# phonism/genrec

Hardware: NVIDIA H100
Metric: hstu_train_sequences_per_sec (higher is better)
Workload: dtype bf16

## Files before the change

### genrec_b200/_lib.py

```python
from __future__ import annotations

import ctypes as C
import os
from typing import Optional

import torch

_HERE = os.path.dirname(os.path.abspath(__file__))
LIB_PATH = os.path.join(_HERE, "libgenrec_b200.so")

c_void_p, c_int, c_float, c_size_t = C.c_void_p, C.c_int, C.c_float, C.c_size_t
c_u64, c_i64, c_u32 = C.c_uint64, C.c_int64, C.c_uint32


class HstuDims(C.Structure):
    _fields_ = [("B", c_int), ("L", c_int), ("D", c_int), ("H", c_int), ("npos", c_int), ("ntime", c_int),
                ("dropout_p", c_float), ("seed", c_u64), ("seed_dev", c_void_p), ("layer_index", c_int)]


class HstuLayerParams(C.Structure):
    _fields_ = [(n, c_void_p) for n in ("proj_w", "proj_b", "pos_table", "time_table", "ln1_g", "ln1_b", "ffn1_w",
                                         "ffn1_b", "ffn2_w", "ffn2_b", "ln2_g", "ln2_b")]


# ... 5 lines not shown
class HstuLayerGrads(C.Structure):
    _fields_ = [(n, c_void_p) for n in ("proj_w", "proj_b", "pos_table", "time_table", "ln1_g", "ln1_b", "ffn1_w",
                                         "ffn1_b", "ffn2_w", "ffn2_b", "ln2_g", "ln2_b")]


class HstuSeq(C.Structure):
    _fields_ = [("bias_index", c_void_p), ("ld_index", c_int), ("has_time", c_int), ("pos_uniform", c_int), ("pos_bucket0", c_int)]


class HstuCache(C.Structure):
    _fields_ = [("B", c_int), ("capacity", c_int), ("num_layers", c_int), ("kv", c_void_p), ("timestamps", c_void_p),
                ("lengths", c_void_p), ("overflow", c_void_p)]


class HstuPool(C.Structure):
    _fields_ = [("max_users", c_int), ("num_layers", c_int), ("page_size", c_int), ("num_pages", c_int), ("max_items", c_int),
                ("kv", c_void_p), ("timestamps", c_void_p), ("page_table", c_void_p), ("lengths", c_void_p), ("overflow", c_void_p),
                ("free_stack", c_void_p), ("free_top", c_void_p), ("errors", c_void_p), ("row_of", c_void_p)]


class SasrecDims(C.Structure):
    _fields_ = [("B", c_int), ("L", c_int), ("D", c_int), ("H", c_int), ("dropout_p", c_float), ("seed", c_u64),
                ("seed_dev", c_void_p), ("layer_index", c_int)]


P = C.POINTER
SIGNATURES = {
    "grb_last_error": (C.c_char_p, []),
    "grb_version": (c_int, []),
    "grb_launch_count": (c_u64, []),
    "grb_check_device": (c_int, [c_int]),
    "grb_set_defer_weight_grads": (c_int, [c_int]),
    "grb_join_deferred": (c_int, [c_void_p]),
    "grb_hstu_layer_saved_bytes": (c_size_t, [P(HstuDims)]),
    "grb_hstu_layer_workspace_bytes": (c_size_t, [P(HstuDims)]),
    "grb_hstu_layer_forward": (c_int, [P(HstuDims), P(HstuLayerParams), P(HstuSeq), c_void_p, c_void_p, c_void_p, c_void_p]),
    "grb_hstu_layer_backward": (c_int, [P(HstuDims), P(HstuLayerParams), P(HstuSeq), c_void_p, c_void_p, c_void_p,
                                        P(HstuLayerGrads), c_void_p, c_void_p]),
    "grb_hstu_bias_index": (c_int, [c_void_p, c_void_p, c_void_p, c_void_p, c_int, c_int, c_int, c_int, c_void_p, c_int, c_void_p]),
    "grb_hstu_attention_scratch_bytes": (c_size_t, [P(HstuDims)]),
    "grb_hstu_attention_forward": (c_int, [P(HstuDims), c_void_p, c_void_p, P(HstuSeq), c_void_p, c_void_p, c_void_p]),
    "grb_hstu_attention_backward": (c_int, [P(HstuDims), c_void_p, c_void_p, P(HstuSeq), c_void_p, c_void_p, c_void_p, c_void_p,
                                            c_void_p, c_void_p, c_void_p, c_void_p]),
    "grb_hstu_cache_append": (c_int, [P(HstuCache), c_void_p, c_void_p, c_int, c_void_p, c_void_p, c_void_p]),
    "grb_hstu_layer_extend_workspace_bytes": (c_size_t, [P(HstuDims), c_int]),
    "grb_hstu_layer_extend": (c_int, [P(HstuDims), P(HstuLayerParams), P(HstuCache), c_int, c_void_p, c_void_p, c_int, c_void_p,
                                      c_void_p, c_void_p, c_void_p, c_void_p]),
    "grb_hstu_pool_append": (c_int, [P(HstuPool), c_void_p, c_int, c_void_p, c_void_p, c_int, c_void_p, c_void_p, c_void_p, c_void_p]),
    "grb_hstu_pool_release": (c_int, [P(HstuPool), c_void_p, c_int, c_void_p, c_int, c_void_p]),
    "grb_hstu_layer_extend_paged_workspace_bytes": (c_size_t, [P(HstuDims), P(HstuPool)]),
    "grb_hstu_layer_extend_paged": (c_int, [P(HstuDims), P(HstuLayerParams), P(HstuPool), c_int, c_void_p, c_void_p, c_void_p, c_int,
                                            c_void_p, c_void_p, c_void_p, c_void_p, c_void_p]),
    "grb_collate_jagged": (c_int, [c_void_p, c_void_p, c_void_p, c_void_p, c_int, c_int, c_void_p, c_void_p, c_void_p, c_void_p]),
    "grb_embed_forward": (c_int, [c_void_p, c_void_p, c_void_p, c_void_p, c_void_p, c_int, c_int, c_int, c_float, c_int,
                                  c_float, c_u64, c_void_p, c_void_p]),
    "grb_embed_backward": (c_int, [c_void_p, c_void_p, c_void_p, c_void_p, c_void_p, c_int, c_int, c_int, c_float, c_int, c_float,
                                   c_u64, c_void_p, c_void_p, c_void_p]),
    "grb_head_workspace_bytes": (c_size_t, [c_int, c_int, c_int]),
    "grb_head_splits": (c_int, [c_int, c_int, c_int, c_int]),
    "grb_head_loss_forward_backward": (c_int, [c_void_p, c_void_p, c_void_p, c_float, c_void_p, c_void_p, c_int, c_int, c_int,
                                               c_void_p, c_void_p, c_void_p, c_void_p, c_void_p, c_void_p, c_void_p]),
    "grb_head_sampled_workspace_bytes": (c_size_t, [c_int, c_int, c_int]),
    "grb_head_sampled_loss_forward_backward": (c_int, [c_void_p, c_void_p, c_void_p, c_float, c_void_p, c_void_p, c_void_p, c_void_p,
                                                       c_int, c_int, c_int, c_int, c_void_p, c_void_p, c_void_p, c_void_p, c_void_p,
                                                       c_void_p, c_void_p]),
    "grb_head_logits": (c_int, [c_void_p, c_void_p, c_void_p, c_float, c_void_p, c_int, c_int, c_int, c_void_p, c_void_p,
# ... 124 lines not shown
```

### genrec_b200/csrc/api.cu

```cuda
#include "../../include/genrec_b200.h"

#include <cstdarg>
#include <cstdio>
#include <cstring>
#include <initializer_list>
#include <mutex>
#include <type_traits>
#include <utility>

#include "attn_hstu.cuh"
#include "attn_hstu_extend.cuh"
#include "attn_sasrec.cuh"
#include "attn_t5.cuh"
#include "beam.cuh"
#include "common.cuh"
#include "dp_adam.cuh"
#include "exact_f32.cuh"
#include "head_candidates.cuh"
#include "head_rank.cuh"
#include "head_topk.cuh"
#include "lazy_adam.cuh"
#include "rowwise.cuh"
#include "rq_argmin.cuh"
#include "rq_sinkhorn.cuh"
// ... 102 lines not shown
    const int need = (T + ROW_THREADS / 32 - 1) / (ROW_THREADS / 32), cap = sm_count() * 3;
    return need < cap ? (need < 1 ? 1 : need) : cap;
}
dim3 colsum_grid(int T, int N) {
    const int cx = (N + 255) / 256, maxy = (T + 63) / 64;
    int cy = (4 * sm_count() + cx - 1) / cx;
    cy = cy > maxy ? maxy : cy;
    return dim3(cx, cy < 1 ? 1 : cy);
}
dim3 cast_colsum_grid(int T, int D) {
    const int cx = (D + 127) / 128, maxy = (T + 31) / 32;
    int cy = (8 * sm_count() + cx - 1) / cx;
    cy = cy > maxy ? maxy : cy;
    return dim3(cx, cy < 1 ? 1 : cy);
}
size_t attn_dw_part_floats(int B, int L, int H) { return (size_t)2 * H * B * ((L + ATT_BLK - 1) / ATT_BLK) * 64; }
struct DetOut {
    float* out;
    int len;
};
int det_finish(const float* part, int ngroups, int nmembers, int W, int gpo, int gstride, int estride, std::initializer_list<DetOut> outs,
               cudaStream_t st) {
    DetFinishArgs f;
    memset(&f, 0, sizeof(f));
    f.part = part; f.ngroups = ngroups; f.nmembers = nmembers; f.W = W; f.gpo = gpo; f.gstride = gstride; f.estride = estride;
    int k = 0;
    for (const DetOut& o : outs) { f.out[k] = o.out; f.len[k] = o.len; ++k; }
    const unsigned blocks = (unsigned)(((size_t)ngroups * W * 32 + 255) / 256);
    launch_k(det_finish_kernel, blocks, 256, 0, st, f);
    GRB_CUDA(cudaGetLastError());
    return 0;
}

cudaError_t gemm_bias_act(int act, const bf16* x, const bf16* w, const float* bias, bf16* z, bf16* a, int M, int N, int K, const Dropout& drop,
                          cudaStream_t st) {
    if (act == 0) return launch_tc_gemm<0>(x, w, M, N, K, K, K, TcEpiBiasAct<0>{bias, N, drop}, z, nullptr, N, sm_count(), st);
    if (act == 1) return launch_tc_gemm<0>(x, w, M, N, K, K, K, TcEpiBiasAct<1>{bias, N, drop}, z, a, N, sm_count(), st);
    return launch_tc_gemm<0>(x, w, M, N, K, K, K, TcEpiBiasAct<2>{bias, N, drop}, z, a, N, sm_count(), st);
}
cudaError_t gemm_bias_res(const bf16* x, const bf16* w, const float* bias, const float* res, const float* row_scale, float* y, int M, int N,
                          int K, const Dropout& drop, cudaStream_t st) {
    return launch_tc_gemm<0>(x, w, M, N, K, K, K, TcEpiBiasResidual{bias, res, row_scale, N, drop}, y, nullptr, N, sm_count(), st);
}
cudaError_t gemm_dact(int act, const bf16* dy, const bf16* w, const bf16* z, bf16* g, int M, int N, int K, const Dropout& drop, cudaStream_t st) {
    if (act == 1) return launch_tc_gemm<1>(dy, w, M, N, K, K, N, TcEpiDAct<1>{z, N, drop}, g, nullptr, N, sm_count(), st);
    return launch_tc_gemm<1>(dy, w, M, N, K, K, N, TcEpiDAct<2>{z, N, drop}, g, nullptr, N, sm_count(), st);
}
cudaError_t gemm_nn_f32(const bf16* A, const bf16* B, float* out, const float* res, float scale, int M, int N, int K, int lda, int ldb,
                        cudaStream_t st) {
    return launch_tc_gemm<1>(A, B, M, N, K, lda, ldb, TcEpiF32{res, N, scale}, out, nullptr, N, sm_count(), st);
}

struct LayerSaved {
    bf16 *xb, *zp, *P, *O, *xn, *z1, *hact;
    float *st1, *x1, *st2;
    size_t bytes;
};
LayerSaved carve_saved(void* base, size_t T, size_t D) {
    LayerSaved s;
    Carver c{static_cast<char*>(base)};
    s.xb = c.take<bf16>(T * D * 2);
    s.zp = c.take<bf16>(T * 4 * D * 2);
    s.P = c.take<bf16>(T * 4 * D * 2);
    s.O = c.take<bf16>(T * D * 2);
    s.st1 = c.take<float>(T * 2 * 4);
    s.x1 = c.take<float>(T * D * 4);
    s.xn = c.take<bf16>(T * D * 2);
    s.st2 = c.take<float>(T * 2 * 4);
    s.z1 = c.take<bf16>(T * 4 * D * 2);
    s.hact = c.take<bf16>(T * 4 * D * 2);
    s.bytes = c.off;
    return s;
}
struct LayerWork {
    bf16 *dyb, *dz1, *dO, *dzp;
    float *dxn, *dx1;
    float *part_tn, *part_colsum, *part_cast, *part_ln, *part_attn;
    size_t bytes;
};
void layer_tn_specs(TnSpec (&specs)[3], const bf16* dyb, const bf16* hact, const bf16* dz1, const bf16* xn, const bf16* dzp, const bf16* xb,
                    float* dw2, float* dw1, float* dwp, int T, int D) {
    specs[0] = {dyb, hact, dw2, D, 4 * D, T, D, 4 * D, 4 * D};
    specs[1] = {dz1, xn, dw1, 4 * D, D, T, 4 * D, D, D};
// ... 110 lines not shown
struct SideStream {
    cudaStream_t s = nullptr;
    cudaEvent_t fork = nullptr, join = nullptr;
    bool ok = false, pending = false;
    template <class F>
    int run(cudaStream_t st, F&& launch) {
        if (!ok) {
            GRB_CUDA(cudaStreamCreateWithFlags(&s, cudaStreamNonBlocking));
            GRB_CUDA(cudaEventCreateWithFlags(&fork, cudaEventDisableTiming));
            GRB_CUDA(cudaEventCreateWithFlags(&join, cudaEventDisableTiming));
            ok = true;
        }
        GRB_CUDA(cudaEventRecord(fork, st));
        GRB_CUDA(cudaStreamWaitEvent(s, fork, 0));
        GRB_TRY(launch(s));
        GRB_CUDA(cudaEventRecord(join, s));
        pending = true;
        return 0;
    }
    int join_into(cudaStream_t st) {
        if (pending) {
            GRB_CUDA(cudaStreamWaitEvent(st, join, 0));
            pending = false;
        }
        return 0;
    }
};
SideStream& attn_side_stream() {
    static thread_local SideStream ss[64];
    return ss[current_device() & 63];
}
std::mutex g_defer_mu;
bool g_defer_on = false;
SideStream& defer_stream() {
    static SideStream ds[64];
    return ds[current_device() & 63];
}
template <class F>
int defer_run(cudaStream_t st, F&& launch) {
    std::lock_guard<std::mutex> lock(g_defer_mu);
    return defer_stream().run(st, launch);
}
int join_pending(cudaStream_t st) {
    std::lock_guard<std::mutex> lock(g_defer_mu);
    return defer_stream().join_into(st);
}
template <class F>
int run_maybe_deferred(cudaStream_t st, F&& launch) {
    if (g_defer_on) return defer_run(st, launch);
    return launch(st);
}

template <int DH>
int launch_hstu_attn_bwd(const HstuAttnArgs& a, cudaStream_t st) {
    dim3 grid((a.L + ATT_BLK - 1) / ATT_BLK, a.H, a.B);
    size_t posb = align_up((size_t)(a.bias.npos * 64 + 1) * 4, 16);
    size_t smem_q = sizeof(AttSmem<DH>) + posb;
    GRB_TRY(set_smem(hstu_attn_bwd_dq_kernel<DH>, smem_q));
    SideStream& ss = attn_side_stream();
    GRB_TRY(ss.run(st, [&](cudaStream_t side) -> int {
        launch_k(hstu_attn_bwd_dq_kernel<DH>, grid, ATT_THREADS, smem_q, side, a);
        GRB_CUDA(cudaGetLastError());
        return 0;
    }));
    const bool has_time = a.bias.wtime != nullptr && a.bias.ntime > 0, pos_uni = a.bias.pos_uniform != 0;
    size_t smem_k = sizeof(AttSmemKV<DH>) + posb +
                    (size_t)4 * (att_time_bins(has_time, pos_uni, a.bias.ntime) + (pos_uni ? 0 : a.bias.npos + 1)) * 32 * sizeof(float);
    const int nmem = (int)(grid.x * grid.z), ngroups = has_time && a.dwtime ? 2 * a.H : a.H;
    GRB_REQUIRE((pos_uni || a.bias.npos <= 64) && a.bias.ntime <= 64, "attention backward: at most 64 position / time buckets");
    auto go = [&](auto kern) -> int {
        GRB_TRY(set_smem(kern, smem_k));
        launch_k(kern, grid, ATT_THREADS, smem_k, st, a, (int)posb);
        return 0;
    };
    if (has_time && pos_uni) GRB_TRY(go(hstu_attn_bwd_dkdv_kernel<DH, true, true>));
    else if (has_time) GRB_TRY(go(hstu_attn_bwd_dkdv_kernel<DH, true, false>));
    else if (pos_uni) GRB_TRY(go(hstu_attn_bwd_dkdv_kernel<DH, false, true>));
    else GRB_TRY(go(hstu_attn_bwd_dkdv_kernel<DH, false, false>));
// ... 175 lines not shown
extern "C" {

const char* grb_last_error(void) { return g_err; }
int grb_version(void) { return 100; }
uint64_t grb_launch_count(void) { return (uint64_t)launch_counter(); }

int grb_check_device(int ordinal) {
    cudaDeviceProp prop;
    cudaError_t e = cudaGetDeviceProperties(&prop, ordinal);
    if (e != cudaSuccess) return fail(GRB_ENODEV, "cudaGetDeviceProperties(%d): %s", ordinal, cudaGetErrorString(e));
    if (prop.major != 9 || prop.minor != 0) return fail(GRB_ENODEV, "device %d is sm_%d%d; this library is built for sm_90a only", ordinal, prop.major, prop.minor);
    return 0;
}

size_t grb_hstu_layer_saved_bytes(const grb_hstu_dims* d) {
    if (check_dims(d)) return 0;
    return carve_saved(nullptr, (size_t)d->B * d->L, d->D).bytes;
}
size_t grb_hstu_layer_workspace_bytes(const grb_hstu_dims* d) {
    if (check_dims(d)) return 0;
    return carve_work(nullptr, d).bytes;
}

int grb_hstu_layer_forward(const grb_hstu_dims* d, const grb_hstu_layer_params* p, const grb_hstu_seq* s, const float* x,
                           float* y, void* saved, void* stream) {
    GRB_TRY(check_dims(d));
    GRB_REQUIRE(x && y && saved, "null argument");
    GRB_TRY(check_layer_params(p));
    GRB_TRY(check_seq(d, s));
    GRB_REQUIRE(aligned16(x) && aligned16(y) && aligned16(saved), "buffers must be 16-byte aligned");
    cudaStream_t st = static_cast<cudaStream_t>(stream);
    const int T = d->B * d->L, D = d->D;
    LayerSaved sv = carve_saved(saved, T, D);

    GRB_TRY(block_steps_in(p, x, sv, T, D, st));
    GRB_TRY(join_pending(st));
    HstuAttnArgs a = make_attn_args(d, p->pos_table, p->time_table, s, sv.P, sv.O);
    GRB_TRY(with_head_dim(D / d->H, [&](auto DH) { return launch_hstu_attn_fwd<DH>(a, st); }));
    return block_steps_out(p, x, y, sv, T, D, make_dropout(d->dropout_p, d->seed, site_of(d->layer_index, SITE_GATE), d->seed_dev),
                           make_dropout(d->dropout_p, d->seed, site_of(d->layer_index, SITE_FFN_HID), d->seed_dev),
                           make_dropout(d->dropout_p, d->seed, site_of(d->layer_index, SITE_FFN_OUT), d->seed_dev), st);
}

int grb_hstu_layer_backward(const grb_hstu_dims* d, const grb_hstu_layer_params* p, const grb_hstu_seq* s, const float* dy,
                            const void* saved, float* dx, const grb_hstu_layer_grads* g, void* workspace, void* stream) {
    GRB_TRY(check_dims(d));
    GRB_REQUIRE(p && dy && saved && dx && g && workspace, "null argument");
    GRB_TRY(check_seq(d, s));
    GRB_REQUIRE(g->proj_w && g->proj_b && g->pos_table && g->ln1_g && g->ln1_b && g->ffn1_w && g->ffn1_b && g->ffn2_w && g->ffn2_b &&
                    g->ln2_g && g->ln2_b, "null gradient pointer");
    GRB_REQUIRE(aligned16(dy) && aligned16(dx) && aligned16(saved) && aligned16(workspace), "buffers must be 16-byte aligned");
    cudaStream_t st = static_cast<cudaStream_t>(stream);
    const int T = d->B * d->L, D = d->D;
    LayerSaved sv = carve_saved(const_cast<void*>(saved), T, D);
    LayerWork w = carve_work(workspace, d);
    const Dropout drop_out = make_dropout(d->dropout_p, d->seed, site_of(d->layer_index, SITE_FFN_OUT), d->seed_dev);
    const Dropout drop_hid = make_dropout(d->dropout_p, d->seed, site_of(d->layer_index, SITE_FFN_HID), d->seed_dev);
    const Dropout drop_gate = make_dropout(d->dropout_p, d->seed, site_of(d->layer_index, SITE_GATE), d->seed_dev);

    GRB_TRY(cast_colsum(dy, w.dyb, T, D, drop_out, g->ffn2_b, w.part_cast, st));
    GRB_CUDA(gemm_dact(1, w.dyb, (const bf16*)p->ffn2_w, sv.z1, w.dz1, T, 4 * D, D, drop_hid, st));
    auto colsum_4d = [&](const bf16* in, float* out) {
        return run_maybe_deferred(st, [&](cudaStream_t s_) -> int { return colsum(in, T, 4 * D, 4 * D, out, w.part_colsum, s_); });
    };
    GRB_TRY(colsum_4d(w.dz1, g->ffn1_b));
    GRB_CUDA(gemm_nn_f32(w.dz1, (const bf16*)p->ffn1_w, w.dxn, nullptr, 1.f, T, D, 4 * D, 4 * D, D, st));
    {
        LnGateBwdArgs a{dy, w.dxn, sv.x1, sv.st1, sv.st2, sv.O, D, sv.P, 4 * D, sv.zp, 4 * D, p->ln1_g, p->ln1_b, p->ln2_g,
                        w.dx1, w.dO, D, w.dzp, 4 * D, g->ln1_g, g->ln1_b, g->ln2_g, g->ln2_b, T, D, drop_gate, w.part_ln};
        GRB_TRY(with_row_dim(D, [&](auto DC) { launch_k(ln_gate_bwd_kernel<DC / 64>, row_grid(T), ROW_THREADS, 0, st, a); }));
        GRB_TRY(det_finish(w.part_ln, 4, row_grid(T), D, 1, 0, 1, {{a.dg1, D}, {a.db1, D}, {a.dg2, D}, {a.db2, D}}, st));
    }
    {
        HstuAttnArgs a = make_attn_args(d, p->pos_table, p->time_table, s, sv.P, sv.O);
        GRB_TRY(set_attn_bwd_args(a, d, s, w.dO, sv.zp, w.dzp, g->pos_table, g->time_table, w.part_attn));
        GRB_TRY(with_head_dim(D / d->H, [&](auto DH) { return launch_hstu_attn_bwd<DH>(a, st); }));
    }
    GRB_TRY(colsum_4d(w.dzp, g->proj_b));
    GRB_CUDA(gemm_nn_f32(w.dzp, (const bf16*)p->proj_w, dx, w.dx1, 1.f, T, D, 4 * D, 4 * D, D, st));
    TnSpec specs[3];
    layer_tn_specs(specs, w.dyb, sv.hact, w.dz1, sv.xn, w.dzp, sv.xb, g->ffn2_w, g->ffn1_w, g->proj_w, T, D);
    return run_maybe_deferred(st, [&](cudaStream_t s_) -> int {
        GRB_CUDA(launch_tc_tn_group(specs, 3, sm_count(), w.part_tn, s_));
        return 0;
    });
}

int grb_hstu_cache_append(const grb_hstu_cache* c, const int64_t* input_ids, const int64_t* timestamps, int n, int32_t* positions,
                          int32_t* last_row, void* stream) {
    GRB_REQUIRE(c && input_ids && positions && last_row, "null argument");
    GRB_REQUIRE(c->timestamps && c->lengths && c->overflow, "null cache pointer");
    GRB_REQUIRE(c->B > 0 && n > 0, "bad shape B=%d n=%d", c->B, n);
    GRB_REQUIRE(c->capacity >= 1 && c->capacity <= 16384, "cache capacity %d out of range [1, 16384]", c->capacity);
    launch_k(hstu_cache_append_kernel, (unsigned)((c->B + 3) / 4), 128, 0, static_cast<cudaStream_t>(stream),
             reinterpret_cast<const long long*>(input_ids), reinterpret_cast<const long long*>(timestamps), (const long long*)nullptr,
             (const int*)nullptr, c->B, n, c->capacity, KvPages{nullptr, 1, c->capacity}, reinterpret_cast<long long*>(c->timestamps),
             c->lengths, c->overflow, positions, last_row);
    GRB_CUDA(cudaGetLastError());
    return 0;
}

int grb_hstu_pool_append(const grb_hstu_pool* pool, const int64_t* users, int B, const int64_t* input_ids, const int64_t* timestamps,
                         int n, int32_t* positions, int32_t* last_row, int32_t* room, void* stream) {
    GRB_TRY(check_pool(pool));
    GRB_REQUIRE(users && input_ids && positions && last_row && room, "null argument");
    GRB_REQUIRE(pool->timestamps && pool->page_table && pool->lengths && pool->overflow && pool->free_stack && pool->free_top &&
                    pool->errors && pool->row_of, "null pool pointer");
    GRB_REQUIRE(B > 0 && n > 0, "bad shape B=%d n=%d", B, n);
    cudaStream_t st = static_cast<cudaStream_t>(stream);
    HstuPoolArgs a = pool_args(pool, users, B);
    a.ids = reinterpret_cast<const long long*>(input_ids); a.n = n;
    a.room = room;
    launch_k(hstu_pool_alloc_kernel, 1, POOL_THREADS, 0, st, a);
    GRB_CUDA(cudaGetLastError());
    launch_k(hstu_cache_append_kernel, (unsigned)((B + 3) / 4), 128, 0, st, reinterpret_cast<const long long*>(input_ids),
             reinterpret_cast<const long long*>(timestamps), reinterpret_cast<const long long*>(users), (const int*)room, B, n,
// ... 46 lines not shown
                                const int64_t* time_thr, const float* x, float* y, void* workspace, void* stream) {
    GRB_TRY(check_pool(pool));
    GRB_TRY(check_extend(d, pool->max_items));
    GRB_REQUIRE(p && users && positions && x && y && workspace && pool->kv && pool->timestamps && pool->page_table, "null argument");
    GRB_REQUIRE(layer >= 0 && layer < pool->num_layers, "layer %d out of range [0, %d)", layer, pool->num_layers);
    ExtendKv kv{static_cast<bf16*>(pool->kv) + (size_t)layer * pool->num_pages * pool->page_size * 2 * d->D,
                reinterpret_cast<const long long*>(pool->timestamps), reinterpret_cast<const long long*>(users),
                KvPages{pool->page_table, pool_pt_ld(pool), pool->page_size}, pool->max_items};
    return layer_extend(d, p, kv, positions, pos_bucket, pos_bucket0, time_thr, x, y, workspace, static_cast<cudaStream_t>(stream));
}

int grb_hstu_bias_index(const int64_t* timestamps, const uint8_t* pad, const int64_t* time_thr, const uint8_t* pos_bucket, int B, int L,
                        int npos, int ntime, uint16_t* out, int ld_index, void* stream) {
    GRB_REQUIRE(pad && time_thr && pos_bucket && out, "null argument");
    GRB_REQUIRE(B > 0 && L > 0 && B <= 65535 && L <= 65535, "bad shape B=%d L=%d", B, L);
    GRB_REQUIRE(ld_index >= L && ld_index % 8 == 0, "ld_index must be a multiple of 8 and >= L");
    GRB_REQUIRE(ntime >= 0 && ntime <= ATT_MAX_BUCKETS && npos >= 1 && npos <= ATT_MAX_BUCKETS, "bucket counts out of range");
    dim3 grid((ld_index + 255) / 256, (L + 7) / 8, B);
    auto go = [&](cudaStream_t s_) -> int {
        launch_k(hstu_bias_index_kernel, grid, 256, 0, s_, reinterpret_cast<const long long*>(timestamps), pad,
                 reinterpret_cast<const long long*>(time_thr), pos_bucket, L, ld_index, npos, ntime, out);
        GRB_CUDA(cudaGetLastError());
        return 0;
    };
    return run_maybe_deferred(static_cast<cudaStream_t>(stream), go);
}

int grb_set_defer_weight_grads(int on) {
    std::lock_guard<std::mutex> lock(g_defer_mu);
    g_defer_on = on != 0;
    return 0;
}
int grb_join_deferred(void* stream) { return join_pending(static_cast<cudaStream_t>(stream)); }

size_t grb_hstu_attention_scratch_bytes(const grb_hstu_dims* d) {
    if (check_dims(d)) return 0;
    return align_up(attn_dw_part_floats(d->B, d->L, d->H) * sizeof(float));
}

int grb_hstu_attention_forward(const grb_hstu_dims* d, const float* pos_table, const float* time_table, const grb_hstu_seq* s,
                               const void* P_bf16, void* O_bf16, void* stream) {
    GRB_TRY(check_dims(d));
    GRB_REQUIRE(pos_table && P_bf16 && O_bf16, "null argument");
    GRB_TRY(check_seq(d, s));
    GRB_REQUIRE(aligned16(P_bf16) && aligned16(O_bf16), "buffers must be 16-byte aligned");
    HstuAttnArgs a = make_attn_args(d, pos_table, time_table, s, (const bf16*)P_bf16, (bf16*)O_bf16);
    return with_head_dim(d->D / d->H, [&](auto DH) { return launch_hstu_attn_fwd<DH>(a, static_cast<cudaStream_t>(stream)); });
}
int grb_hstu_attention_backward(const grb_hstu_dims* d, const float* pos_table, const float* time_table, const grb_hstu_seq* s,
                                const void* P_bf16, const void* zp_bf16, const void* dO_bf16, void* dzp_bf16, float* dpos_table,
                                float* dtime_table, void* scratch, void* stream) {
    GRB_TRY(check_dims(d));
    GRB_REQUIRE(pos_table && P_bf16 && dO_bf16 && dzp_bf16 && dpos_table && scratch, "null argument");
    GRB_TRY(check_seq(d, s));
    GRB_REQUIRE(aligned16(P_bf16) && aligned16(dO_bf16) && aligned16(dzp_bf16) && aligned16(scratch) && (zp_bf16 == nullptr || aligned16(zp_bf16)),
                "buffers must be 16-byte aligned");
    HstuAttnArgs a = make_attn_args(d, pos_table, time_table, s, (const bf16*)P_bf16, nullptr);
    GRB_TRY(set_attn_bwd_args(a, d, s, (const bf16*)dO_bf16, (const bf16*)zp_bf16, (bf16*)dzp_bf16, dpos_table, dtime_table,
                              static_cast<float*>(scratch)));
    return with_head_dim(d->D / d->H, [&](auto DH) { return launch_hstu_attn_bwd<DH>(a, static_cast<cudaStream_t>(stream)); });
}

int grb_collate_jagged(const int64_t* items, const int64_t* stamps, const int64_t* offsets, const int64_t* targets, int B, int L,
                       int64_t* out_input_ids, int64_t* out_targets, int64_t* out_timestamps, void* stream) {
    GRB_REQUIRE(items && offsets && targets && out_input_ids && out_targets, "null argument");
    GRB_REQUIRE(B > 0 && L > 0, "bad shape B=%d L=%d", B, L);
    const size_t n = (size_t)B * L;
    launch_k(collate_jagged_kernel, (unsigned)((n + 255) / 256), 256, 0, static_cast<cudaStream_t>(stream), reinterpret_cast<const long long*>(items),
             reinterpret_cast<const long long*>(stamps), reinterpret_cast<const long long*>(offsets), reinterpret_cast<const long long*>(targets), B, L,
             reinterpret_cast<long long*>(out_input_ids), reinterpret_cast<long long*>(out_targets), reinterpret_cast<long long*>(out_timestamps));
    GRB_CUDA(cudaGetLastError());
    return 0;
}

int grb_embed_forward(const int64_t* ids, const float* table, const float* pos_table, float* x, uint8_t* pad, int B, int L, int D,
                      float scale, int mask_pad_rows, float dropout_p, uint64_t seed, const uint64_t* seed_dev, void* stream) {
    GRB_REQUIRE(ids && table && x, "null argument");
    GRB_REQUIRE(B > 0 && L > 0 && D > 0 && D % 4 == 0, "bad shape");
    EmbedArgs a{reinterpret_cast<const long long*>(ids), table, pos_table, x, pad, B * L, L, D, scale, mask_pad_rows,
                make_dropout(dropout_p, seed, SITE_EMBED, seed_dev)};
    launch_k(embed_fwd_kernel, row_grid(B * L), ROW_THREADS, 0, static_cast<cudaStream_t>(stream), a);
    GRB_CUDA(cudaGetLastError());
    return 0;
}
int grb_embed_backward(const int64_t* ids, const int64_t* order, const float* dx, float* dtable, float* dpos_table, int B, int L, int D,
                       float scale, int mask_pad_rows, float dropout_p, uint64_t seed, const uint64_t* seed_dev, float* scratch, void* stream) {
    GRB_REQUIRE(ids && order && dx && dtable && scratch, "null argument");
    GRB_REQUIRE(D <= 128 * EMB_MAX_CH, "embedding backward supports D <= %d", 128 * EMB_MAX_CH);
    GRB_REQUIRE(D % 4 == 0 && aligned16(dx) && aligned16(dtable) && aligned16(scratch) && (dpos_table == nullptr || aligned16(dpos_table)),
                "embedding backward needs D %% 4 == 0 and 16-byte aligned buffers");
    EmbedBwdArgs a{reinterpret_cast<const long long*>(ids), dx, dtable, dpos_table, B * L, L, D, scale, mask_pad_rows,
                   make_dropout(dropout_p, seed, SITE_EMBED, seed_dev), reinterpret_cast<const long long*>(order)};
    const EmbedPieceArgs pa{a, scratch};
    launch_k(embed_bwd_piece_kernel, row_grid((B * L + 31) / 32), ROW_THREADS, 0, static_cast<cudaStream_t>(stream), pa);
    GRB_CUDA(cudaGetLastError());
    launch_k(embed_bwd_run_kernel, row_grid(B * L), ROW_THREADS, 0, static_cast<cudaStream_t>(stream), pa);
    GRB_CUDA(cudaGetLastError());
    if (dpos_table) {
        launch_k(embed_bwd_pos_kernel, L < 8 * sm_count() ? L : 8 * sm_count(), ROW_THREADS, 0, static_cast<cudaStream_t>(stream), a);
        GRB_CUDA(cudaGetLastError());
    }
    return 0;
}

namespace {
struct HeadCommon {
    bf16* xf; float* stf; float* dxf; float* scal;
    float* row_loss;
    float* shift;
    float* part_ln;
};
void carve_head_common(Carver& c, HeadCommon& h, size_t T, size_t D) {
    h.xf = c.take<bf16>(T * D * 2);
    h.stf = c.take<float>(T * 2 * 4);
    h.dxf = c.take<float>(T * D * 4);
    h.scal = c.take<float>(64);
    h.row_loss = c.take<float>(T * 4);
    h.shift = c.take<float>(T * 4);
    h.part_ln = c.take<float>((size_t)2 * row_bwd_grid((int)T) * D * 4);
}
struct HeadWork : HeadCommon {
    bf16* logits;
    float* logits32;
    float* part_tn;
    int *ce_rsched, *ce_tsched;
    float *ce_rcarry, *ce_tcarry;
// ... 32 lines not shown

size_t grb_head_workspace_bytes(int T, int D, int C) { return carve_head(nullptr, T, D, C).bytes; }
int grb_head_splits(int T, int D, int C, int table) {
    const HeadWork h = carve_head(nullptr, T, D, C);
    return table ? h.tseg : h.rseg;
}

int grb_head_loss_forward_backward(const float* x, const float* ln_g, const float* ln_b, float ln_eps, const void* table_bf16,
                                   const int64_t* targets, int T, int D, int C, float* loss, float* dx, float* dtable, float* dln_g,
                                   float* dln_b, void* workspace, void* stream) {
    GRB_REQUIRE(x && ln_g && ln_b && table_bf16 && targets && loss && workspace, "null argument");
    GRB_REQUIRE(T > 0 && C > 1 && (D == 64 || D == 128 || D == 256), "bad shape T=%d D=%d C=%d", T, D, C);
    const bool want_grad = dx != nullptr;
    GRB_REQUIRE(!want_grad || (dtable && dln_g && dln_b), "null gradient pointer");
    cudaStream_t st = static_cast<cudaStream_t>(stream);
    HeadWork h = carve_head(workspace, T, D, C);
    const bool count_aside = g_defer_on;
    auto count = [&](cudaStream_t s_) -> int {
        launch_k(ce_count_kernel, 1, 1024, 0, s_, reinterpret_cast<const long long*>(targets), T, h.scal, loss);
        GRB_CUDA(cudaGetLastError());
        return 0;
    };
    if (count_aside) GRB_TRY(defer_run(st, count));
    GRB_TRY(head_ln_forward(x, ln_g, ln_b, ln_eps, h.xf, h.stf, T, D, st));
    if (count_aside) GRB_TRY(join_pending(st));
    else GRB_TRY(count(st));
    if (head_fused(D)) {
        CeArgs ca{reinterpret_cast<const long long*>(targets), h.scal, T, C, want_grad ? h.dxf : nullptr, h.shift, h.row_loss, dtable,
                  h.rseg, h.tseg, h.ce_rsched, h.ce_tsched, h.ce_rcarry, h.ce_tcarry};
        GRB_CUDA(with_ce_dim(D, [&](auto DC) { return launch_tc_ce<DC>(h.xf, (const bf16*)table_bf16, ca, sm_count(), st); }));
        launch_k(ce_loss_sum_kernel, 1, 1024, 0, st, (const float*)h.row_loss, T, loss);
        GRB_CUDA(cudaGetLastError());
        if (!want_grad) return 0;
        GRB_TRY(run_maybe_deferred(st, [&](cudaStream_t s_) -> int {
            GRB_CUDA(with_ce_dim(D, [&](auto DC) { return launch_ce_table<DC>(h.xf, (const bf16*)table_bf16, ca, sm_count(), s_); }));
            return 0;
        }));
    } else {
        GRB_CUDA((launch_tc_gemm<0>(h.xf, (const bf16*)table_bf16, T, C, D, D, D, TcEpiF32{nullptr, h.ldl, 1.f}, h.logits32, nullptr, h.ldl,
                                    sm_count(), st)));
        if (h.ldl / 8 <= 256 * 8)
            launch_k(ce_fwd_bwd_vec_kernel<8>, T, 256, 0, st, h.logits, h.ldl, C, reinterpret_cast<const long long*>(targets), h.scal, h.row_loss, want_grad ? 1 : 0,
                     (const float*)h.logits32);
        else
            launch_k(ce_fwd_bwd_kernel, T, 256, 0, st, h.logits, h.ldl, C, reinterpret_cast<const long long*>(targets), h.scal, h.row_loss, want_grad ? 1 : 0,
                     (const float*)h.logits32);
        GRB_CUDA(cudaGetLastError());
        launch_k(ce_loss_sum_kernel, 1, 1024, 0, st, (const float*)h.row_loss, T, loss);
        GRB_CUDA(cudaGetLastError());
        if (!want_grad) return 0;
        GRB_CUDA(gemm_nn_f32(h.logits, (const bf16*)table_bf16, h.dxf, nullptr, 1.f, T, D, C, h.ldl, D, st));
        TnSpec spec{h.logits, h.xf, dtable, C, D, T, h.ldl, D, D};
        GRB_TRY(run_maybe_deferred(st, [&](cudaStream_t s_) -> int {
            GRB_CUDA(launch_tc_tn_group(&spec, 1, sm_count(), h.part_tn, s_));
            return 0;
        }));
    }
    return head_ln_backward(h, x, ln_g, dx, dln_g, dln_b, T, D, st);
}

namespace {
struct SampledWork : HeadCommon {
    bf16* Es; float* bias; int* sid;
    float *ztgt, *gtgt;
    float* part; int ks;
    int Npad;
    size_t bytes;
};
SampledWork carve_sampled(void* base, size_t T, size_t D, size_t N) {
    SampledWork h;
    Carver c{static_cast<char*>(base)};
    h.Npad = (int)((N + 63) / 64 * 64);
    h.ks = sce_table_splits((int)T, h.Npad, sm_count());
    carve_head_common(c, h, T, D);
    h.Es = c.take<bf16>((size_t)h.Npad * D * 2);
    h.bias = c.take<float>((size_t)h.Npad * 4);
    h.sid = c.take<int>((size_t)h.Npad * 4);
    h.ztgt = c.take<float>(T * 4);
    h.gtgt = c.take<float>(T * 4);
    h.part = c.take<float>((size_t)h.ks * h.Npad * D * 4);
    h.bytes = c.off;
    return h;
}
int check_sampled_shape(int T, int D, int N) {
    GRB_REQUIRE(T >= 1, "sampled head: T=%d must be >= 1", T);
    GRB_REQUIRE(D == 64 || D == 128, "sampled head: D=%d is not supported (D must be 64 or 128; D = 256 is served by the full head only)", D);
    GRB_REQUIRE(N >= 1 && N <= SCE_MAX_N, "sampled head: N=%d negatives, must be 1 .. %d", N, SCE_MAX_N);
    return 0;
}
// ... 348 lines not shown
    float *part_colsum, *part_tn;
    size_t bytes;
};
TnSpec linear_dw_spec(const void* dy_bf16, const void* x_bf16, float* dw, int T, int N, int K) {
    return TnSpec{(const bf16*)dy_bf16, (const bf16*)x_bf16, dw, N, K, T, N, K, K};
}
LinearBwdWork carve_linear_bwd(void* base, int T, int N, int K) {
    LinearBwdWork w;
    Carver c{static_cast<char*>(base)};
    const dim3 cg = colsum_grid(T, N);
    w.part_colsum = c.take<float>((size_t)cg.x * cg.y * 256 * 4);
    const TnSpec spec = linear_dw_spec(nullptr, nullptr, nullptr, T, N, K);
    w.part_tn = c.take<float>(tn_part_floats(&spec, 1, sm_count()) * 4);
    w.bytes = c.off;
    return w;
}
}

size_t grb_linear_backward_workspace_bytes(int T, int N, int K) {
    if (T <= 0 || N <= 0 || K <= 0) return 0;
    return carve_linear_bwd(nullptr, T, N, K).bytes;
}
int grb_linear_backward(const void* dy_bf16, const void* w_bf16, const void* x_bf16, int T, int N, int K, float* dx_f32,
                        const float* dx_residual, float* dw, float* db, void* workspace, void* stream) {
    GRB_REQUIRE(dy_bf16 && w_bf16, "null argument");
    GRB_REQUIRE(T > 0 && N % 8 == 0 && K % 8 == 0, "N and K must be multiples of 8");
    GRB_REQUIRE(workspace || (!dw && !db), "workspace is null");
    cudaStream_t st = static_cast<cudaStream_t>(stream);
    const LinearBwdWork w = carve_linear_bwd(workspace, T, N, K);
    if (db) GRB_TRY(colsum((const bf16*)dy_bf16, T, N, N, db, w.part_colsum, st));
    if (dw) {
        GRB_REQUIRE(x_bf16, "x is null");
        const TnSpec spec = linear_dw_spec(dy_bf16, x_bf16, dw, T, N, K);
        GRB_CUDA(launch_tc_tn_group(&spec, 1, sm_count(), w.part_tn, st));
    }
    if (dx_f32) {
        GRB_CUDA(gemm_nn_f32((const bf16*)dy_bf16, (const bf16*)w_bf16, dx_f32, dx_residual, 1.f, T, K, N, N, K, st));
    }
    return 0;
}

int grb_linear_dact_backward(const void* dy_bf16, const void* w_bf16, const void* z_bf16, int T, int N, int K, int act, float dropout_p,
                             uint64_t seed, const uint64_t* seed_dev, uint32_t site, void* g_bf16, void* stream) {
    GRB_REQUIRE(dy_bf16 && w_bf16 && z_bf16 && g_bf16, "null argument");
    GRB_REQUIRE(T > 0 && N % 8 == 0 && K % 8 == 0 && (act == 1 || act == 2), "bad argument");
    GRB_CUDA(gemm_dact(act, (const bf16*)dy_bf16, (const bf16*)w_bf16, (const bf16*)z_bf16, (bf16*)g_bf16, T, K, N,
                       make_dropout(dropout_p, seed, site, seed_dev), static_cast<cudaStream_t>(stream)));
    return 0;
}
int grb_cast_rows_f32_to_bf16(const float* in, void* out_bf16, int T, int D, const float* row_scale, float dropout_p, uint64_t seed,
                              const uint64_t* seed_dev, uint32_t site, void* stream) {
    GRB_REQUIRE(in && out_bf16 && T > 0 && D > 0 && D % 4 == 0, "bad argument");
    return cast_bf16(in, (bf16*)out_bf16, (size_t)T * D, D, make_dropout(dropout_p, seed, site, seed_dev), row_scale,
                     static_cast<cudaStream_t>(stream));
}

int grb_layernorm_forward(const float* x, const float* g, const float* b, float eps, int T, int D, void* y_bf16, float* y_f32,
                          float* stats, void* stream) {
    GRB_REQUIRE(x && g && b && (y_bf16 || y_f32), "null argument");
    LnFwdArgs a{x, g, b, (bf16*)y_bf16, y_f32, stats, T, D, eps};
    cudaStream_t st = static_cast<cudaStream_t>(stream);
    return with_row_dim(D, [&](auto DC) { launch_k(ln_fwd_kernel<DC / 64>, row_grid(T), ROW_THREADS, 0, st, a); });
}
size_t grb_layernorm_backward_workspace_bytes(int T, int D) {
    if (T <= 0 || D <= 0) return 0;
    return (size_t)2 * row_bwd_grid(T) * D * 4;
}
// ... 489 lines not shown
```

### genrec_b200/csrc/tc_tn_group.cuh

```cuda
#pragma once
#include "tc_gemm.cuh"

namespace grb {

constexpr int TN_MAX_PROBLEMS = 4;

struct TnProblem {
    int M, N, K;
    int num_m, num_n, splits, kb_total, kb_per_split;
    int work_begin;
    int part_begin;
    float* out;
    int ldo;
};
struct TnGroupParams {
    CUtensorMap tmA[TN_MAX_PROBLEMS];
    CUtensorMap tmB[TN_MAX_PROBLEMS];
    TnProblem p[TN_MAX_PROBLEMS];
    int nprob;
    int total_work;
    float* part;
};


// ... 149 lines not shown
    memset(&P, 0, sizeof(P));
    P.nprob = n;
    double total = 0;
    for (int i = 0; i < n; ++i) total += (double)specs[i].M * specs[i].N * specs[i].K;
    int work = 0, parts = 0;
    for (int i = 0; i < n; ++i) {
        const TnSpec& s = specs[i];
        TnProblem& q = P.p[i];
        q.M = s.M; q.N = s.N; q.K = s.K; q.out = s.out; q.ldo = s.ldo;
        q.num_m = (s.M + TC_BM - 1) / TC_BM;
        q.num_n = (s.N + TC_BN - 1) / TC_BN;
        q.kb_total = (s.K + TC_BK - 1) / TC_BK;
        const int tiles = q.num_m * q.num_n;
        int want_items = (int)(2.0 * num_sms * ((double)s.M * s.N * s.K / total) + 0.5);
        int splits = (want_items + tiles - 1) / tiles;
        if (splits < 1) splits = 1;
        int max_splits = q.kb_total / 4 > 0 ? q.kb_total / 4 : 1;
        if (splits > max_splits) splits = max_splits;
        q.kb_per_split = (q.kb_total + splits - 1) / splits;
        q.splits = (q.kb_total + q.kb_per_split - 1) / q.kb_per_split;
        q.work_begin = work;
        q.part_begin = q.splits > 1 ? parts : -1;
        work += tiles * q.splits;
        if (q.splits > 1) parts += tiles * q.splits;
    }
    P.total_work = work;
    return (size_t)parts * (TC_BM * TC_BN);
}
inline size_t tn_part_floats(const TnSpec* specs, int n, int num_sms) {
    TnGroupParams P;
    return n < 1 || n > TN_MAX_PROBLEMS ? 0 : tn_plan(P, specs, n, num_sms);
}

inline cudaError_t launch_tc_tn_group(const TnSpec* specs, int n, int num_sms, float* part, cudaStream_t st) {
    if (n < 1 || n > TN_MAX_PROBLEMS) return cudaErrorInvalidValue;
    TnGroupParams P;
    const size_t need = tn_plan(P, specs, n, num_sms);
    if (need > 0 && part == nullptr) return cudaErrorInvalidValue;
    P.part = part;
    for (int i = 0; i < n; ++i) {
        const TnSpec& s = specs[i];
        if (!make_tmap_bf16(&P.tmA[i], s.A, s.K, s.M, s.lda, 64, TC_BK) || !make_tmap_bf16(&P.tmB[i], s.B, s.K, s.N, s.ldb, 64, TC_BK))
            return cudaErrorInvalidValue;
    }
    const int work = P.total_work;
    cudaError_t e = set_max_smem(tc_tn_group_kernel, TN_SMEM_BYTES);
    if (e != cudaSuccess) return e;
    int grid = work < num_sms ? work : num_sms;
    launch_k(tc_tn_group_kernel, grid, TC_THREADS, TN_SMEM_BYTES, st, P);
    e = cudaGetLastError();
    if (e != cudaSuccess) return e;
    int tiles = 0;
    for (int i = 0; i < n; ++i)
        if (P.p[i].splits > 1) tiles += P.p[i].num_m * P.p[i].num_n;
    if (tiles == 0) return cudaSuccess;
    launch_k(tn_finish_kernel, tiles * TN_FINISH_SLABS, 256, 0, st, P);
    return cudaGetLastError();
}

}
```

### include/genrec_b200.h

```cpp
#ifndef GENREC_B200_H
#define GENREC_B200_H

#include <stddef.h>
#include <stdint.h>

#ifdef __cplusplus
extern "C" {
#endif

#define GRB_OK 0
#define GRB_EINVAL (-1)
#define GRB_ECUDA (-2)
#define GRB_ENODEV (-3)

const char* grb_last_error(void);
int grb_version(void);
uint64_t grb_launch_count(void);
int grb_check_device(int ordinal);

typedef struct {
    int B, L, D, H;
    int npos, ntime;
    float dropout_p;
    uint64_t seed;
// ... 11 lines not shown
    const void* ffn1_w;
    const float* ffn1_b;
    const void* ffn2_w;
    const float* ffn2_b;
    const float* ln2_g;
    const float* ln2_b;
} grb_hstu_layer_params;

typedef struct {
    float* proj_w; float* proj_b; float* pos_table; float* time_table;
    float* ln1_g; float* ln1_b; float* ffn1_w; float* ffn1_b; float* ffn2_w; float* ffn2_b; float* ln2_g; float* ln2_b;
} grb_hstu_layer_grads;

typedef struct {
    const uint16_t* bias_index;
    int ld_index;
    int has_time;
    int pos_uniform;
    int pos_bucket0;
} grb_hstu_seq;

size_t grb_hstu_attention_scratch_bytes(const grb_hstu_dims* d);
int grb_hstu_attention_forward(const grb_hstu_dims* d, const float* pos_table, const float* time_table, const grb_hstu_seq* s,
                               const void* P_bf16, void* O_bf16, void* stream);
int grb_hstu_attention_backward(const grb_hstu_dims* d, const float* pos_table, const float* time_table, const grb_hstu_seq* s,
                                const void* P_bf16, const void* zp_bf16, const void* dO_bf16, void* dzp_bf16, float* dpos_table,
                                float* dtime_table, void* scratch, void* stream);

int grb_hstu_bias_index(const int64_t* timestamps, const uint8_t* pad, const int64_t* time_thr, const uint8_t* pos_bucket, int B,
                        int L, int npos, int ntime, uint16_t* out, int ld_index, void* stream);

int grb_set_defer_weight_grads(int on);
int grb_join_deferred(void* stream);

size_t grb_hstu_layer_saved_bytes(const grb_hstu_dims* d);
size_t grb_hstu_layer_workspace_bytes(const grb_hstu_dims* d);
int grb_hstu_layer_forward(const grb_hstu_dims* d, const grb_hstu_layer_params* p, const grb_hstu_seq* s,
                           const float* x, float* y, void* saved, void* stream);
int grb_hstu_layer_backward(const grb_hstu_dims* d, const grb_hstu_layer_params* p, const grb_hstu_seq* s,
                            const float* dy, const void* saved, float* dx, const grb_hstu_layer_grads* g,
                            void* workspace, void* stream);

typedef struct {
    int B, capacity, num_layers;
    void* kv;
    int64_t* timestamps;
    int32_t* lengths;
    uint8_t* overflow;
} grb_hstu_cache;
int grb_hstu_cache_append(const grb_hstu_cache* c, const int64_t* input_ids, const int64_t* timestamps, int n, int32_t* positions,
                          int32_t* last_row, void* stream);
size_t grb_hstu_layer_extend_workspace_bytes(const grb_hstu_dims* d, int capacity);
int grb_hstu_layer_extend(const grb_hstu_dims* d, const grb_hstu_layer_params* p, const grb_hstu_cache* c, int layer,
                          const int32_t* positions, const uint8_t* pos_bucket, int pos_bucket0, const int64_t* time_thr,
                          const float* x, float* y, void* workspace, void* stream);

typedef struct {
    int max_users, num_layers;
    int page_size;
    int num_pages;
    int max_items;
    void* kv;
    int64_t* timestamps;
    int32_t* page_table;
    int32_t* lengths;
    uint8_t* overflow;
// ... 149 lines not shown
```

Before: 40590.

## Partition SMs between main stream and deferred side-stream weight-grad kernels

Adds an SM budget for deferred side-stream work (the CE table gradient and TN weight-grad groups). The budget is sized from a cost model comparing table-pass time with the remaining block-chain time, and the main-stream GEMMs now launch on the SMs left over. An event makes embedding backward wait for the table gradient. The aim is real overlap between the deferred table gradient and the backward chain instead of both competing for every SM. The risk is that the main GEMMs run on fewer SMs and that the hard-coded cost constants are miscalibrated for H100.

```diff
diff --git a/genrec_b200/_lib.py b/genrec_b200/_lib.py
--- a/genrec_b200/_lib.py
+++ b/genrec_b200/_lib.py
@@ -61,6 +61,7 @@
     "grb_check_device": (c_int, [c_int]),
     "grb_set_defer_weight_grads": (c_int, [c_int]),
     "grb_join_deferred": (c_int, [c_void_p]),
+    "grb_set_side_sm_budget": (c_int, [c_int]),
     "grb_hstu_layer_saved_bytes": (c_size_t, [P(HstuDims)]),
     "grb_hstu_layer_workspace_bytes": (c_size_t, [P(HstuDims)]),
     "grb_hstu_layer_forward": (c_int, [P(HstuDims), P(HstuLayerParams), P(HstuSeq), c_void_p, c_void_p, c_void_p, c_void_p]),
diff --git a/genrec_b200/csrc/api.cu b/genrec_b200/csrc/api.cu
--- a/genrec_b200/csrc/api.cu
+++ b/genrec_b200/csrc/api.cu
@@ -158,23 +158,25 @@
     return 0;
 }
 
+int main_sms();
+
 cudaError_t gemm_bias_act(int act, const bf16* x, const bf16* w, const float* bias, bf16* z, bf16* a, int M, int N, int K, const Dropout& drop,
                           cudaStream_t st) {
-    if (act == 0) return launch_tc_gemm<0>(x, w, M, N, K, K, K, TcEpiBiasAct<0>{bias, N, drop}, z, nullptr, N, sm_count(), st);
-    if (act == 1) return launch_tc_gemm<0>(x, w, M, N, K, K, K, TcEpiBiasAct<1>{bias, N, drop}, z, a, N, sm_count(), st);
-    return launch_tc_gemm<0>(x, w, M, N, K, K, K, TcEpiBiasAct<2>{bias, N, drop}, z, a, N, sm_count(), st);
+    if (act == 0) return launch_tc_gemm<0>(x, w, M, N, K, K, K, TcEpiBiasAct<0>{bias, N, drop}, z, nullptr, N, main_sms(), st);
+    if (act == 1) return launch_tc_gemm<0>(x, w, M, N, K, K, K, TcEpiBiasAct<1>{bias, N, drop}, z, a, N, main_sms(), st);
+    return launch_tc_gemm<0>(x, w, M, N, K, K, K, TcEpiBiasAct<2>{bias, N, drop}, z, a, N, main_sms(), st);
 }
 cudaError_t gemm_bias_res(const bf16* x, const bf16* w, const float* bias, const float* res, const float* row_scale, float* y, int M, int N,
                           int K, const Dropout& drop, cudaStream_t st) {
-    return launch_tc_gemm<0>(x, w, M, N, K, K, K, TcEpiBiasResidual{bias, res, row_scale, N, drop}, y, nullptr, N, sm_count(), st);
+    return launch_tc_gemm<0>(x, w, M, N, K, K, K, TcEpiBiasResidual{bias, res, row_scale, N, drop}, y, nullptr, N, main_sms(), st);
 }
 cudaError_t gemm_dact(int act, const bf16* dy, const bf16* w, const bf16* z, bf16* g, int M, int N, int K, const Dropout& drop, cudaStream_t st) {
-    if (act == 1) return launch_tc_gemm<1>(dy, w, M, N, K, K, N, TcEpiDAct<1>{z, N, drop}, g, nullptr, N, sm_count(), st);
-    return launch_tc_gemm<1>(dy, w, M, N, K, K, N, TcEpiDAct<2>{z, N, drop}, g, nullptr, N, sm_count(), st);
+    if (act == 1) return launch_tc_gemm<1>(dy, w, M, N, K, K, N, TcEpiDAct<1>{z, N, drop}, g, nullptr, N, main_sms(), st);
+    return launch_tc_gemm<1>(dy, w, M, N, K, K, N, TcEpiDAct<2>{z, N, drop}, g, nullptr, N, main_sms(), st);
 }
 cudaError_t gemm_nn_f32(const bf16* A, const bf16* B, float* out, const float* res, float scale, int M, int N, int K, int lda, int ldb,
                         cudaStream_t st) {
-    return launch_tc_gemm<1>(A, B, M, N, K, lda, ldb, TcEpiF32{res, N, scale}, out, nullptr, N, sm_count(), st);
+    return launch_tc_gemm<1>(A, B, M, N, K, lda, ldb, TcEpiF32{res, N, scale}, out, nullptr, N, main_sms(), st);
 }
 
 struct LayerSaved {
@@ -351,8 +353,16 @@
 }
 std::mutex g_defer_mu;
 bool g_defer_on = false;
-SideStream& defer_stream() {
-    static SideStream ds[64];
+int g_side_budget = 0;
+struct DeferStream : SideStream {
+    cudaEvent_t table = nullptr;
+    bool table_pending = false;
+    int budget = 0;
+    int blocks = 0;
+    double chain_us = 0;
+};
+DeferStream& defer_stream() {
+    static DeferStream ds[64];
     return ds[current_device() & 63];
 }
 template <class F>
@@ -362,7 +372,62 @@
 }
 int join_pending(cudaStream_t st) {
     std::lock_guard<std::mutex> lock(g_defer_mu);
-    return defer_stream().join_into(st);
+    DeferStream& ds = defer_stream();
+    ds.budget = 0;
+    ds.table_pending = false;
+    return ds.join_into(st);
+}
+double table_pass_us(double T, double C, double D) { return 1.03e-8 * T * C * D; }
+double block_chain_us(double T, double L, double D) { return 3.75e-7 * T * D * D + 2.18e-7 * T * L * D; }
+int table_budget(double table_us) {
+    const int S = sm_count();
+    int b = g_side_budget;
+    if (b <= 0) {
+        const DeferStream& ds = defer_stream();
+        if (ds.blocks < 2) return 0;
+        b = (int)(S * table_us / (ds.chain_us * (ds.blocks - 1) / ds.blocks) + 0.999);
+    }
+    b = b < S - 1 ? b : S - 1;
+    return b < 1 ? 1 : b;
+}
+template <class F>
+int defer_run_sized(cudaStream_t st, double table_us, F&& launch) {
+    std::lock_guard<std::mutex> lock(g_defer_mu);
+    DeferStream& ds = defer_stream();
+    if (table_us > 0) ds.budget = table_budget(table_us);
+    const int ctas = table_us > 0 && ds.budget > 0 ? ds.budget : sm_count();
+    return ds.run(st, [&](cudaStream_t s) { return launch(s, ctas); });
+}
+void lift_budget() {
+    std::lock_guard<std::mutex> lock(g_defer_mu);
+    if (g_side_budget <= 0) defer_stream().budget = 0;
+}
+void count_block(const grb_hstu_dims* d) {
+    std::lock_guard<std::mutex> lock(g_defer_mu);
+    DeferStream& ds = defer_stream();
+    if (d->layer_index == 0) { ds.blocks = 0; ds.chain_us = 0; }
+    ds.blocks += 1;
+    ds.chain_us += block_chain_us((double)d->B * d->L, d->L, d->D);
+}
+int mark_table(cudaStream_t s) {
+    DeferStream& ds = defer_stream();
+    if (!ds.table) GRB_CUDA(cudaEventCreateWithFlags(&ds.table, cudaEventDisableTiming));
+    GRB_CUDA(cudaEventRecord(ds.table, s));
+    ds.table_pending = true;
+    return 0;
+}
+int wait_table(cudaStream_t st) {
+    std::lock_guard<std::mutex> lock(g_defer_mu);
+    DeferStream& ds = defer_stream();
+    if (ds.table_pending) {
+        GRB_CUDA(cudaStreamWaitEvent(st, ds.table, 0));
+        ds.table_pending = false;
+    }
+    return 0;
+}
+int main_sms() {
+    std::lock_guard<std::mutex> lock(g_defer_mu);
+    return sm_count() - defer_stream().budget;
 }
 template <class F>
 int run_maybe_deferred(cudaStream_t st, F&& launch) {
@@ -604,6 +669,7 @@
     cudaStream_t st = static_cast<cudaStream_t>(stream);
     const int T = d->B * d->L, D = d->D;
     LayerSaved sv = carve_saved(saved, T, D);
+    count_block(d);
 
     GRB_TRY(block_steps_in(p, x, sv, T, D, st));
     GRB_TRY(join_pending(st));
@@ -626,6 +692,7 @@
     const int T = d->B * d->L, D = d->D;
     LayerSaved sv = carve_saved(const_cast<void*>(saved), T, D);
     LayerWork w = carve_work(workspace, d);
+    if (d->layer_index == 0) lift_budget();
     const Dropout drop_out = make_dropout(d->dropout_p, d->seed, site_of(d->layer_index, SITE_FFN_OUT), d->seed_dev);
     const Dropout drop_hid = make_dropout(d->dropout_p, d->seed, site_of(d->layer_index, SITE_FFN_HID), d->seed_dev);
     const Dropout drop_gate = make_dropout(d->dropout_p, d->seed, site_of(d->layer_index, SITE_GATE), d->seed_dev);
@@ -652,8 +719,12 @@
     GRB_CUDA(gemm_nn_f32(w.dzp, (const bf16*)p->proj_w, dx, w.dx1, 1.f, T, D, 4 * D, 4 * D, D, st));
     TnSpec specs[3];
     layer_tn_specs(specs, w.dyb, sv.hact, w.dz1, sv.xn, w.dzp, sv.xb, g->ffn2_w, g->ffn1_w, g->proj_w, T, D);
-    return run_maybe_deferred(st, [&](cudaStream_t s_) -> int {
-        GRB_CUDA(launch_tc_tn_group(specs, 3, sm_count(), w.part_tn, s_));
+    if (!g_defer_on) {
+        GRB_CUDA(launch_tc_tn_group(specs, 3, sm_count(), sm_count(), w.part_tn, st));
+        return 0;
+    }
+    return defer_run_sized(st, 0.0, [&](cudaStream_t s_, int ctas) -> int {
+        GRB_CUDA(launch_tc_tn_group(specs, 3, sm_count(), ctas, w.part_tn, s_));
         return 0;
     });
 }
@@ -766,6 +837,12 @@
     return 0;
 }
 int grb_join_deferred(void* stream) { return join_pending(static_cast<cudaStream_t>(stream)); }
+int grb_set_side_sm_budget(int ctas) {
+    GRB_REQUIRE(ctas >= 0, "side SM budget %d must be >= 0 (0: the default rule)", ctas);
+    std::lock_guard<std::mutex> lock(g_defer_mu);
+    g_side_budget = ctas;
+    return 0;
+}
 
 size_t grb_hstu_attention_scratch_bytes(const grb_hstu_dims* d) {
     if (check_dims(d)) return 0;
@@ -826,6 +903,7 @@
     EmbedBwdArgs a{reinterpret_cast<const long long*>(ids), dx, dtable, dpos_table, B * L, L, D, scale, mask_pad_rows,
                    make_dropout(dropout_p, seed, SITE_EMBED, seed_dev), reinterpret_cast<const long long*>(order)};
     const EmbedPieceArgs pa{a, scratch};
+    GRB_TRY(wait_table(static_cast<cudaStream_t>(stream)));
     launch_k(embed_bwd_piece_kernel, row_grid((B * L + 31) / 32), ROW_THREADS, 0, static_cast<cudaStream_t>(stream), pa);
     GRB_CUDA(cudaGetLastError());
     launch_k(embed_bwd_run_kernel, row_grid(B * L), ROW_THREADS, 0, static_cast<cudaStream_t>(stream), pa);
@@ -924,10 +1002,14 @@
         launch_k(ce_loss_sum_kernel, 1, 1024, 0, st, (const float*)h.row_loss, T, loss);
         GRB_CUDA(cudaGetLastError());
         if (!want_grad) return 0;
-        GRB_TRY(run_maybe_deferred(st, [&](cudaStream_t s_) -> int {
-            GRB_CUDA(with_ce_dim(D, [&](auto DC) { return launch_ce_table<DC>(h.xf, (const bf16*)table_bf16, ca, sm_count(), s_); }));
-            return 0;
-        }));
+        if (!g_defer_on) {
+            GRB_CUDA(with_ce_dim(D, [&](auto DC) { return launch_ce_table<DC>(h.xf, (const bf16*)table_bf16, ca, sm_count(), st); }));
+        } else {
+            GRB_TRY(defer_run_sized(st, table_pass_us(T, C, D), [&](cudaStream_t s_, int ctas) -> int {
+                GRB_CUDA(with_ce_dim(D, [&](auto DC) { return launch_ce_table<DC>(h.xf, (const bf16*)table_bf16, ca, ctas, s_); }));
+                return mark_table(s_);
+            }));
+        }
     } else {
         GRB_CUDA((launch_tc_gemm<0>(h.xf, (const bf16*)table_bf16, T, C, D, D, D, TcEpiF32{nullptr, h.ldl, 1.f}, h.logits32, nullptr, h.ldl,
                                     sm_count(), st)));
@@ -943,10 +1025,14 @@
         if (!want_grad) return 0;
         GRB_CUDA(gemm_nn_f32(h.logits, (const bf16*)table_bf16, h.dxf, nullptr, 1.f, T, D, C, h.ldl, D, st));
         TnSpec spec{h.logits, h.xf, dtable, C, D, T, h.ldl, D, D};
-        GRB_TRY(run_maybe_deferred(st, [&](cudaStream_t s_) -> int {
-            GRB_CUDA(launch_tc_tn_group(&spec, 1, sm_count(), h.part_tn, s_));
-            return 0;
-        }));
+        if (!g_defer_on) {
+            GRB_CUDA(launch_tc_tn_group(&spec, 1, sm_count(), sm_count(), h.part_tn, st));
+        } else {
+            GRB_TRY(defer_run_sized(st, 0.0, [&](cudaStream_t s_, int ctas) -> int {
+                GRB_CUDA(launch_tc_tn_group(&spec, 1, sm_count(), ctas, h.part_tn, s_));
+                return mark_table(s_);
+            }));
+        }
     }
     return head_ln_backward(h, x, ln_g, dx, dln_g, dln_b, T, D, st);
 }
@@ -1361,7 +1447,7 @@
     if (dw) {
         GRB_REQUIRE(x_bf16, "x is null");
         const TnSpec spec = linear_dw_spec(dy_bf16, x_bf16, dw, T, N, K);
-        GRB_CUDA(launch_tc_tn_group(&spec, 1, sm_count(), w.part_tn, st));
+        GRB_CUDA(launch_tc_tn_group(&spec, 1, sm_count(), sm_count(), w.part_tn, st));
     }
     if (dx_f32) {
         GRB_CUDA(gemm_nn_f32((const bf16*)dy_bf16, (const bf16*)w_bf16, dx_f32, dx_residual, 1.f, T, K, N, N, K, st));
diff --git a/genrec_b200/csrc/tc_tn_group.cuh b/genrec_b200/csrc/tc_tn_group.cuh
--- a/genrec_b200/csrc/tc_tn_group.cuh
+++ b/genrec_b200/csrc/tc_tn_group.cuh
@@ -205,7 +205,7 @@
     return n < 1 || n > TN_MAX_PROBLEMS ? 0 : tn_plan(P, specs, n, num_sms);
 }
 
-inline cudaError_t launch_tc_tn_group(const TnSpec* specs, int n, int num_sms, float* part, cudaStream_t st) {
+inline cudaError_t launch_tc_tn_group(const TnSpec* specs, int n, int num_sms, int ctas, float* part, cudaStream_t st) {
     if (n < 1 || n > TN_MAX_PROBLEMS) return cudaErrorInvalidValue;
     TnGroupParams P;
     const size_t need = tn_plan(P, specs, n, num_sms);
@@ -219,7 +219,7 @@
     const int work = P.total_work;
     cudaError_t e = set_max_smem(tc_tn_group_kernel, TN_SMEM_BYTES);
     if (e != cudaSuccess) return e;
-    int grid = work < num_sms ? work : num_sms;
+    int grid = work < ctas ? work : ctas;
     launch_k(tc_tn_group_kernel, grid, TC_THREADS, TN_SMEM_BYTES, st, P);
     e = cudaGetLastError();
     if (e != cudaSuccess) return e;
diff --git a/include/genrec_b200.h b/include/genrec_b200.h
--- a/include/genrec_b200.h
+++ b/include/genrec_b200.h
@@ -67,6 +67,7 @@
 
 int grb_set_defer_weight_grads(int on);
 int grb_join_deferred(void* stream);
+int grb_set_side_sm_budget(int ctas);
 
 size_t grb_hstu_layer_saved_bytes(const grb_hstu_dims* d);
 size_t grb_hstu_layer_workspace_bytes(const grb_hstu_dims* d);
```

After: 41050, median of 6. 1.1% higher.
